# broadinstitute/gatk-bwamem-jni

Measured on AMD Instinct MI355X. Metric: 150bp reads aligned/sec vs GRCh38-scale reference (1/2/4/8 MI355X), higher is better.
Workload: dtype u8/int32/int64; 1 GPU; 10000000 x 150bp single-end synthetic reads per GPU vs synthetic GRCh38-scale genome (3100000000 bp, 24 contigs, 5% diverged repeats), full index in HBM; reads_per_gpu=10000000, read_len=150, genome_bp=3100000000, genome=iid, response_bytes=542940344, parallelism=read-sharded x1, no collectives, hip_hw_queues=4, paired_end=False

## Files before the change

### gatk-bwamem-jni_amd/csrc/bwamem_types.h

```cpp
#pragma once
#include <stdint.h>
#include <stddef.h>
#include <hip/hip_runtime.h>

struct MemOpt {
    int a, b;
    int o_del, e_del;
    int o_ins, e_ins;
    int pen_unpaired;
    int pen_clip5, pen_clip3;
    int w;
    int zdrop;
    uint64_t max_mem_intv;
    int T;
    int flag;
    int min_seed_len;
    int min_chain_weight;
    int max_chain_extend;
    float split_factor;
    int split_width;
    int max_occ;
    int max_chain_gap;
    int n_threads;
    int chunk_size;
    float mask_level;
    float drop_ratio;
    float XA_drop_ratio;
    float mask_level_redun;
    float mapQ_coef_len;
    int mapQ_coef_fac;
    int max_ins;
    int max_matesw;
    int max_XA_hits, max_XA_hits_alt;
    int8_t mat[25];
};
static_assert(sizeof(MemOpt) == 168, "mem_opt_t ABI (BwaMemAligner.java:137)");

struct MemPestat { int low, high; int failed; double avg, std; };
static_assert(sizeof(MemPestat) == 32, "mem_pestat_t ABI");

struct PairTab { const double* t; int64_t lo[4]; int32_t n[4], off[4]; };

enum {
    MEM_F_PE = 0x2, MEM_F_NOPAIRING = 0x4, MEM_F_ALL = 0x8, MEM_F_NO_MULTI = 0x10,
    MEM_F_NO_RESCUE = 0x20, MEM_F_PRIMARY5 = 0x800
};

struct DevIndex {
    const uint4* occ;
    const uint32_t* sa_lo;
    const uint8_t*  sa_hi;
    const uint8_t*  pac;
    const int64_t*  ann_offset;
    const int32_t*  ann_len;
    const int32_t*  ann_is_alt;
    const int32_t*  ann_name_off;
    const char*     names;
    const double*   log_tab;
    uint64_t primary, L2[5], seq_len;
    int64_t  l_pac;
    int32_t  n_seqs, sa_intv, log_tab_n, sa_shift;
    int32_t  n_cu, lds_bytes;
};

struct Intv { uint64_t x0, x1, size, info; };

struct Seed { int64_t rbeg; int32_t qbeg, len, score, next; };

struct Chain {
    int64_t pos;
    int32_t n, first, rid;
    uint32_t w;
    int32_t kept, is_alt;
    int32_t seed0;
    int32_t last;
    float frac_rep;
    int32_t pad_;
};

struct AlnReg {
    int64_t rb, re;
    int32_t qb, qe;
    int32_t rid;
    int32_t score, truesc, sub, alt_sc, csub, sub_n, w, seedcov, secondary, secondary_all, seedlen0;
    int32_t n_comp, is_alt;
    float frac_rep;
    int32_t pad_;
    uint64_t hash;
};

struct SwJob { int64_t rb; int32_t read, tag, l_ms, is_rev, tlen, xtra, q_off, pad_; };
struct KswR { int score, te, qe, score2, te2, tb, qb; };

struct DevCounters {
    unsigned long long n_ext, n_lf, n_sa, n_dp_cells, n_ref_bases, n_reads;
    unsigned long long dbg[10];
};

enum { ERR_INTV_CAP = 1, ERR_OUT_CAP = 2, ERR_CIGAR_CAP = 4, ERR_LONG_READ = 8, ERR_SCRATCH = 16, ERR_BTREE = 32, ERR_BAD_REG = 64, ERR_JOB_CAP = 128, ERR_ZPOOL = 256, ERR_RESCUE_CAP = 512 };

#define BT_NODE_INTS 40

struct TileView {
    int32_t n_reads;
    int32_t max_len;
    int64_t read_id0;
    const int64_t* seq_off;
    uint8_t* seq;
    int32_t intv_cap;
    Intv* intv;
    int32_t* n_intv;
    Intv* smem_scratch;
    int32_t smem_cap;
    int32_t* l_rep;
    int32_t* n_seeds;
    int64_t* seed_off;
// ... 31 lines not shown
```

### gatk-bwamem-jni_amd/csrc/k_seed.hip

```cpp
#include "dev_common.h"
#include "wave_ops.h"
#include "kernels.h"

DEV uint32_t mask16(int n)
{
    n = n < 0 ? 0 : n > 16 ? 16 : n;
    return (uint32_t)(0x5555555500000000ull >> (n << 1));
}
DEV void cnt_word_m(uint32_t x, uint32_t m, uint32_t& c1, uint32_t& c2, uint32_t& c3)
{
    const uint32_t lo = x & m, hi = (x >> 1) & m;
    c3 += __popc(hi & lo);
    c2 += __popc(hi & ~lo);
    c1 += __popc(~hi & lo);
}
DEV void extend_sm(const DevIndex& ix, uint64_t x0, uint64_t x1, uint64_t size, int c, bool is_back, uint64_t& o0, uint64_t& o1, uint64_t& osz)
{
    const uint64_t xa = is_back ? x0 : x1, xb = is_back ? x1 : x0;
    const uint64_t k = xa - 1, l = xa - 1 + size;
    const uint64_t kk = k - (k >= ix.primary), ll = l - (l >= ix.primary);
    const uint64_t bk = kk >> 6, bl = ll >> 6;
    const uint4* pk = ix.occ + 2 * bk;
    const uint4* pl = ix.occ + 2 * bl;
    const uint4 ck = pk[0], sk = pk[1], cl = pl[0], sl = pl[1];
// ... 23 lines not shown
    uint32_t *v0, *v1, *v2;
    uint16_t* v2n;
    uint4* spill;
    int K, spill_cap;
    bool narrow;
    static __device__ uint32_t pack2(uint64_t x0, uint64_t size, int end) { return (uint32_t)(x0 >> 32) | (uint32_t)(size >> 32) << 5 | (uint32_t)end << 10; }
    __device__ uint32_t hi_get(int e) const {
        const int s = (e & (K - 1)) * 64;
        if (!narrow) return v2[s];
        const uint32_t h = v2n[s];
        return (h & 7u) | (h >> 3 & 7u) << 5 | (h >> 6) << 10;
    }
    __device__ void hi_put(int e, uint32_t w2) {
        const int s = (e & (K - 1)) * 64;
        if (!narrow) v2[s] = w2;
        else v2n[s] = (uint16_t)((w2 & 7u) | (w2 >> 5 & 7u) << 3 | (w2 >> 10) << 6);
    }
    __device__ bool push(int e, uint64_t x0, uint64_t size, int end) {
        const int s = (e & (K - 1)) * 64;
        if (e >= K) {
            if (e - K >= spill_cap) return false;
            uint4 t; t.x = v0[s]; t.y = v1[s]; t.z = hi_get(e); t.w = 0;
            spill[(size_t)(e - K) * 64] = t;
        }
        v0[s] = (uint32_t)x0; v1[s] = (uint32_t)size; hi_put(e, pack2(x0, size, end));
        return true;
    }
    __device__ void put(int e, int n, uint64_t x0, uint64_t size, int end) {
        if (e >= n - K) { const int s = (e & (K - 1)) * 64; v0[s] = (uint32_t)x0; v1[s] = (uint32_t)size; hi_put(e, pack2(x0, size, end)); }
        else { uint4 t; t.x = (uint32_t)x0; t.y = (uint32_t)size; t.z = pack2(x0, size, end); t.w = 0; spill[(size_t)e * 64] = t; }
    }
    __device__ void get(int e, int n, uint64_t& x0, uint64_t& size, int& end) const {
        uint32_t a, b, w2;
        if (e >= n - K) { const int s = (e & (K - 1)) * 64; a = v0[s]; b = v1[s]; w2 = hi_get(e); }
        else { const uint4 t = spill[(size_t)e * 64]; a = t.x; b = t.y; w2 = t.z; }
        x0 = (uint64_t)(w2 & 31) << 32 | a; size = (uint64_t)(w2 >> 5 & 31) << 32 | b; end = (int)(w2 >> 10);
    }
};

__global__ void k_encode(uint8_t* seq, int64_t n_bytes)
{
    int64_t i = (int64_t)blockIdx.x * blockDim.x + threadIdx.x;
    int64_t stride = (int64_t)gridDim.x * blockDim.x;
    for (; i < n_bytes; i += stride) {
        uint8_t c = seq[i];
        if (c >= 4) {
            uint8_t u = c & 0xdf;
            c = u == 'A' ? 0 : u == 'C' ? 1 : u == 'G' ? 2 : u == 'T' ? 3 : 4;
            seq[i] = c;
        }
    }
}

enum { S_IDLE = 0, S_NEXT = 1, S_FWD = 2, S_BWD = 3, S_P3 = 4 };
#define SEED_EL_CAP 4

template <bool LDSQ>
__global__ void __launch_bounds__(64) k_seed(DevIndex ix, MemOpt opt, TileView tv, int K, int refill_min, int narrow)
{
    HIP_DYNAMIC_SHARED(uint32_t, lds)
    const int lane = threadIdx.x;
    CandStack V;
    V.narrow = narrow != 0;
    V.v0 = lds + lane; V.v1 = V.v0 + K * 64; V.v2 = V.v1 + K * 64; V.K = K;
    V.v2n = (uint16_t*)(lds + 2 * K * 64) + lane;
    V.spill = (uint4*)tv.smem_scratch + (size_t)blockIdx.x * tv.smem_cap * 64 + lane; V.spill_cap = tv.smem_cap;
    uint32_t* el = lds + (narrow ? 5 * K * 32 : 3 * K * 64) + lane;
    uint32_t* sq = el + SEED_EL_CAP * 64;
    unsigned int* work = (unsigned int*)(tv.err + 8);
    const int min_seed_len = opt.min_seed_len;
    const int split_len = (int)(opt.min_seed_len * opt.split_factor + .499);
    const uint64_t max_intv3 = (uint64_t)(int64_t)(int)opt.max_mem_intv;

    int st = S_IDLE, r = 0, len = 0, pass = 1, x = 0, sx = 0, i = 0, k2 = 0, old_n = 0, mem_n = 0;
    int nf = 0, lo = 0, rd = 0, wr = 0, c = -1, ret = 0, end = 0, n_el = 0;
    uint64_t min_intv = 1, last_start = 0, last_sz = 0, ik0 = 0, ik1 = 0, iks = 0;
    bool any = false, ovf = false, exhausted = false, el_ok = true;
    const uint8_t* qg = tv.seq;
    Intv* mem = tv.intv;
    uint32_t n_ext = 0;

    uint64_t qwin = 0;
    const uint8_t* qwin_at = nullptr;
    auto qat_g = [&](int p) -> int {
        const uint8_t* a = qg + p;
        const uint8_t* al = a - ((uintptr_t)a & 7);
        if (al != qwin_at) { qwin_at = al; qwin = *(const uint64_t*)al; }
        return (int)(qwin >> (((uintptr_t)a & 7) << 3) & 0xffu);
    };
#define QAT(p) (LDSQ ? (int)(sq[((p) >> 3) * 64] >> (((p) & 7) << 2) & 15u) : qat_g(p))
#define FINISH() do { fin = true; st = S_IDLE; } while (0)
#define MEM_PUSH(X0, SZ, INFO) do { if (mem_n >= tv.intv_cap) ovf = true; else { Intv v_; v_.x0 = (X0); v_.x1 = 0; v_.size = (SZ); v_.info = (INFO); mem[mem_n++] = v_; } } while (0)
#define PUSH_IK() do { if (V.push(nf, ik0, iks, end)) ++nf; else ovf = true; } while (0)
#define BEGIN_BWD() do { ret = end; lo = 0; rd = wr = nf - 1; i = sx - 1; c = i >= 0 ? QAT(i) : 4; c = c < 4 ? c : -1; st = S_BWD; } while (0)

    for (;;) {
        bool fin = false;
        const unsigned long long idle = __ballot(st == S_IDLE);
        if (idle != 0ull && !exhausted && (__popcll(idle) >= refill_min || idle == ~0ull)) {
            const int n_need = __popcll(idle);
            unsigned int base = 0;
            if (lane == 0) base = atomicAdd(work, (unsigned int)n_need);
            base = (unsigned int)__shfl((int)base, 0);
            if (base + (unsigned int)n_need >= (unsigned int)tv.n_reads) exhausted = true;
            bool fresh = false;
            if (st == S_IDLE) {
                const unsigned int cand = base + (unsigned int)__popcll(idle & ((1ull << lane) - 1ull));
                if (cand < (unsigned int)tv.n_reads) {
                    r = (int)cand; fresh = true;
                    const int64_t off = tv.seq_off[r];
                    len = (int)(tv.seq_off[r + 1] - off - 1);
                    qg = tv.seq + off;
                    mem = tv.intv + (size_t)r * tv.intv_cap;
                    mem_n = 0; ovf = false; pass = 1; x = 0; st = S_NEXT; n_el = 0; el_ok = true;
                }
            }
            if (LDSQ) {
                unsigned long long got = __ballot(fresh);
                while (got) {
                    const int l = __ffsll((long long)got) - 1;
                    got &= got - 1ull;
                    const int rr = __shfl(r, l);
                    const int64_t off = tv.seq_off[rr];
                    const int nb = (int)(tv.seq_off[rr + 1] - off) - 1;
                    for (int k = lane; k * 8 < nb; k += 64) {
                        uint32_t wd = 0;
                        uint32_t by[8];
#pragma unroll
                        for (int b = 0; b < 8; ++b) { const int pos = k * 8 + b; by[b] = tv.seq[off + (pos < nb ? pos : nb)]; }
#pragma unroll
                        for (int b = 0; b < 8; ++b) wd |= (k * 8 + b < nb ? by[b] & 15u : 4u) << (b << 2);
                        sq[k * 64 + (l - lane)] = wd;
                    }
                }
                __syncthreads();
            }
            if (fresh && len < min_seed_len) { tv.n_intv[r] = 0; st = S_IDLE; }
        }
        if (__ballot(st != S_IDLE) == 0ull) break;

        if (st == S_NEXT) {
            int nx = -1;
            bool p3 = false;
            uint64_t nmin = 1;
            if (pass == 1) {
                if (x >= len) { pass = 2; old_n = mem_n; k2 = 0; }
                else if (QAT(x) > 3) ++x;
                else nx = x;
            } else if (pass == 2 && el_ok) {
                if (k2 >= n_el) { pass = 3; x = 0; if (!(opt.max_mem_intv > 0)) FINISH(); }
                else {
                    const uint32_t wd = el[k2 * 64];
                    const int m = (int)(wd & 0x1ffffu);
                    if (QAT(m) > 3) ++k2;
                    else { nx = m; nmin = (uint64_t)(wd >> 17) + 1; }
                }
            } else if (pass == 2) {
                if (k2 >= old_n) { pass = 3; x = 0; if (!(opt.max_mem_intv > 0)) FINISH(); }
                else {
                    const uint64_t psz = mem[k2].size, pinfo = mem[k2].info;
                    const int s0 = (int)(pinfo >> 32), e0 = (int)(int32_t)pinfo;
                    if (e0 - s0 < split_len || psz > (uint64_t)(int64_t)opt.split_width) ++k2;
                    else {
                        const int m = (s0 + e0) >> 1;
                        if (QAT(m) > 3) ++k2;
                        else { nx = m; nmin = psz + 1; }
                    }
                }
            } else {
                if (x >= len) FINISH();
                else if (QAT(x) > 3) ++x;
                else { nx = x; p3 = true; }
            }
            if (nx >= 0) {
                const int b = QAT(nx);
                const uint64_t lb = b == 0 ? ix.L2[0] : b == 1 ? ix.L2[1] : b == 2 ? ix.L2[2] : ix.L2[3];
                const uint64_t lb1 = b == 0 ? ix.L2[1] : b == 1 ? ix.L2[2] : b == 2 ? ix.L2[3] : ix.L2[4];
                const uint64_t lc = b == 0 ? ix.L2[3] : b == 1 ? ix.L2[2] : b == 2 ? ix.L2[1] : ix.L2[0];
                ik0 = lb + 1; iks = lb1 - lb; ik1 = lc + 1;
                sx = nx; i = sx + 1;
                if (p3) st = S_P3;
                else { min_intv = nmin; end = sx + 1; nf = 0; any = false; st = S_FWD; }
            }
        }

        bool need = false, bw = false, back = false;
        int rc = 0, pend = 0;
        uint64_t r0 = 0, r1 = 0, rs = 0;
        bool fwd_end = false;
        if (st == S_FWD || st == S_P3) {
            const int cq = i < len ? QAT(i) : 4;
            if (cq < 4) { need = true; rc = 3 - cq; r0 = ik0; r1 = ik1; rs = iks; }
            else if (st == S_FWD) fwd_end = true;
            else { x = i < len ? i + 1 : len; st = S_NEXT; }
        }
        if (st == S_BWD) {
            V.get(rd, nf, r0, rs, pend);
            bw = true;
            if (c >= 0) { need = true; back = true; rc = c; }
        }

        uint64_t o0 = 0, o1 = 0, os = 0, em0 = 0, ems = 0, emi = 0;
        bool emit = false;
        if (need) { extend_sm(ix, r0, r1, rs, rc, back, o0, o1, os); ++n_ext; }

        if (bw) {
            if (!need || os < min_intv) {
                if (wr == nf - 1 && (!any || (uint64_t)(i + 1) < last_start)) {
                    any = true; last_start = (uint64_t)(i + 1);
                    if (pend - (i + 1) >= min_seed_len) {
                        emit = true; em0 = r0; ems = rs; emi = (uint64_t)(i + 1) << 32 | (uint32_t)pend;
                        if (pass == 1 && pend - (i + 1) >= split_len && rs <= (uint64_t)(int64_t)opt.split_width) {
                            if (n_el < SEED_EL_CAP && rs < 32768u) el[n_el * 64] = (uint32_t)((i + 1 + pend) >> 1) | (uint32_t)rs << 17;
                            else el_ok = false;
                            ++n_el;
                        }
                    }
                }
            } else if (wr == nf - 1 || os != last_sz) {
                V.put(wr, nf, o0, os, pend); --wr; last_sz = os;
            }
            --rd;
            if (rd < lo) {
                if (wr == nf - 1) { if (pass == 1) x = ret; else ++k2; st = S_NEXT; }
                else { lo = wr + 1; rd = wr = nf - 1; --i; c = i >= 0 ? QAT(i) : 4; c = c < 4 ? c : -1; }
            }
        } else if (st == S_FWD && (need || fwd_end)) {
            const bool push = fwd_end || os != iks;
            const bool stop = fwd_end || (push && os < min_intv);
            if (push) PUSH_IK();
            if (stop) BEGIN_BWD();
            else { ik0 = o0; ik1 = o1; iks = os; end = i + 1; ++i; }
        } else if (need) {
            if (os < max_intv3 && i - sx >= min_seed_len) {
                if (os > 0) { emit = true; em0 = o0; ems = os; emi = (uint64_t)sx << 32 | (uint32_t)(i + 1); }
                x = i + 1; st = S_NEXT;
            } else { ik0 = o0; ik1 = o1; iks = os; ++i; }
        }
        if (emit) MEM_PUSH(em0, ems, emi);
        if (ovf) FINISH();
        if (fin) {
            tv.n_intv[r] = ovf ? 0 : mem_n;
            if (ovf) atomicOr(tv.err, ERR_INTV_CAP);
        }
    }
#undef QAT
#undef FINISH
#undef MEM_PUSH
#undef PUSH_IK
#undef BEGIN_BWD
    unsigned long long tot = n_ext;
    for (int o = 32; o > 0; o >>= 1) tot += __shfl_down(tot, o);
    if (lane == 0) { count_add(&tv.cnt->n_ext, tot); }
}

__global__ void k_seed_fin(MemOpt opt, TileView tv)
{
    const int r = blockIdx.x * blockDim.x + threadIdx.x;
    if (r >= tv.n_reads) return;
    Intv* a = tv.intv + (size_t)r * tv.intv_cap;
    const int n = tv.n_intv[r];
    for (int i = 1; i < n; ++i) {
        Intv t = a[i];
        int j = i;
        while (j > 0 && a[j - 1].info > t.info) { a[j] = a[j - 1]; --j; }
        a[j] = t;
    }
    int n_seeds = 0, l_rep = 0, b = 0, e = 0;
    int32_t* iso = tv.intv_seed_off + (size_t)r * tv.intv_cap;
    for (int i = 0; i < n; ++i) {
        const Intv p = a[i];
        const int sb = (int)(p.info >> 32), se = (int)(uint32_t)p.info;
        iso[i] = n_seeds;
        {
            int64_t step = p.size > (uint64_t)(int64_t)opt.max_occ ? (int64_t)(p.size / (uint64_t)opt.max_occ) : 1;
            int64_t c = ((int64_t)p.size + step - 1) / step;
            n_seeds += (int)(c < opt.max_occ ? c : opt.max_occ);
        }
        if (p.size <= (uint64_t)(int64_t)opt.max_occ) continue;
        if (sb > e) { l_rep += e - b; b = sb; e = se; }
        else e = e > se ? e : se;
    }
    l_rep += e - b;
    tv.n_seeds[r] = n_seeds;
    tv.l_rep[r] = l_rep;
}

__global__ void __launch_bounds__(1024) k_scan(const int32_t* in, int64_t* out, int n)
{
    __shared__ int64_t wtot[2][16];
    const int t = threadIdx.x, lane = t & 63, wv = t >> 6;
    int64_t carry = 0;
    int ph = 0;
    for (int base = 0; base < n; base += 4096, ph ^= 1) {
        const int i0 = base + t * 4;
        int v0 = 0, v1 = 0, v2 = 0, v3 = 0;
        if (i0 + 3 < n) { const int4 q = *(const int4*)(in + i0); v0 = q.x; v1 = q.y; v2 = q.z; v3 = q.w; }
        else { if (i0 < n) v0 = in[i0]; if (i0 + 1 < n) v1 = in[i0 + 1]; if (i0 + 2 < n) v2 = in[i0 + 2]; }
        const int64_t sum = (int64_t)v0 + v1 + v2 + v3;
        int64_t incl = sum;
        for (int o = 1; o < 64; o <<= 1) { int64_t u = __shfl_up(incl, o); if (lane >= o) incl += u; }
        if (lane == 63) wtot[ph][wv] = incl;
        __syncthreads();
        int64_t pre = carry, tot = 0;
        for (int w = 0; w < 16; ++w) { const int64_t x = wtot[ph][w]; if (w < wv) pre += x; tot += x; }
        int64_t run = pre + incl - sum;
        if (i0 < n) out[i0] = run;
        run += v0; if (i0 + 1 < n) out[i0 + 1] = run;
        run += v1; if (i0 + 2 < n) out[i0 + 2] = run;
        run += v2; if (i0 + 3 < n) out[i0 + 3] = run;
        carry += tot;
    }
    if (t == 0) out[n] = carry;
}

DEV int64_t block_excl_scan_256(int64_t v, int64_t* lds4, int64_t& total)
{
    const int lane = threadIdx.x & 63, wv = threadIdx.x >> 6;
    int64_t incl = v;
    for (int o = 1; o < 64; o <<= 1) { int64_t u = __shfl_up(incl, o); if (lane >= o) incl += u; }
    if (lane == 63) lds4[wv] = incl;
    __syncthreads();
// ... 274 lines not shown
```

### gatk-bwamem-jni_amd/csrc/kernels.h

```cpp
#pragma once
#include <hip/hip_runtime.h>
#include "bwamem_types.h"
#include "bam_encode.h"
#include "bam_sort.h"
#include "bam_dup.h"
#include "fastq_parse.h"

void launch_build_occ64(hipStream_t st, const uint32_t* bwt, uint64_t n_blocks, uint4* occ);
void launch_sa_densify(hipStream_t st, const DevIndex& ix, const uint64_t* sa_src, uint64_t n_src, int src_intv, uint32_t* lo, uint8_t* hi, int32_t* err);
void launch_encode(hipStream_t st, uint8_t* seq, int64_t n_bytes);
void launch_unpack_pac(hipStream_t st, const DevIndex& ix, int64_t start, int64_t n, uint8_t* dst);
void launch_seed(hipStream_t st, const DevIndex& ix, const MemOpt& opt, const TileView& tv);
size_t scan_tmp_bytes(int64_t n);
void launch_scan(hipStream_t st, const int32_t* in, int64_t* out, int n, int64_t* tmp);
void launch_order(hipStream_t st, const int32_t* n_seeds, int n, int32_t* bins64, int32_t* order);
size_t nul_tmp_bytes(int64_t n_bytes);
void launch_nul_offsets(hipStream_t st, const uint8_t* seq, int64_t n_bytes, int64_t* off, int64_t n_reads_max, int64_t* n_found, void* tmp);
void launch_sa(hipStream_t st, const DevIndex& ix, const MemOpt& opt, const TileView& tv, int64_t n_occ);
void launch_chain(hipStream_t st, const DevIndex& ix, const MemOpt& opt, const TileView& tv, Chain* chain_store);
bool rescore_needed(const MemOpt& opt, const TileView& tv);
void launch_rescore(hipStream_t st, const DevIndex& ix, const MemOpt& opt, const TileView& tv, void* jobs, void* results, int32_t* first_num, int32_t* cnt, int cap);
size_t extend_lds_bytes(const MemOpt& opt, int max_len);
void launch_extend(hipStream_t st, const DevIndex& ix, const MemOpt& opt, const TileView& tv);
void launch_post1(hipStream_t st, const DevIndex& ix, const MemOpt& opt, const TileView& tv);
void launch_final_prep(hipStream_t st, const DevIndex& ix, const MemOpt& opt, const TileView& tv);
size_t gcigar_slab_bytes(const MemOpt& opt, int max_len);
int gcigar_slab_grid(const DevIndex& ix, int n_jobs);
void launch_gcigar(hipStream_t st, const DevIndex& ix, const MemOpt& opt, const TileView& tv, int n_jobs, const void* jobs, void* outs, uint32_t* cig_pool, int cig_cap,
                   uint8_t* zpool, unsigned long long zpool_cap, unsigned long long* zpool_cur, uint8_t* slabs, size_t slab_bytes, int* queue);
void launch_final_se(hipStream_t st, const DevIndex& ix, const MemOpt& opt, const TileView& tv, const void* job_out, const uint32_t* job_cig, int cig_cap);
void launch_pack(hipStream_t st, const TileView& tv, uint8_t* dst);
void launch_bam_size(hipStream_t st, const BamTile& t);
void launch_bam_emit(hipStream_t st, const BamTile& t);
void launch_qual_check(hipStream_t st, const uint8_t* raw, const uint8_t* qual, const int64_t* raw_off, int n_reads, int32_t* err);
void launch_mate_names(hipStream_t st, const uint8_t* names, const int64_t* name_off, int n_pairs, int32_t* err);
void launch_fastq_count(hipStream_t st, const uint8_t* text, int64_t n, int32_t* counts);
void launch_fastq_starts(hipStream_t st, const FastqText& t);
void launch_fastq_records(hipStream_t st, const FastqText& t, const FastqOut& o);
void launch_fastq_copy(hipStream_t st, const FastqText& t, const FastqOut& o, int max_len);
int bgzf_grid(int n_cu, int64_t n_blocks);
size_t bgzf_token_bytes(int grid);
void launch_bgzf_deflate(hipStream_t st, const uint8_t* src, int64_t n, int n_blocks, int grid, uint8_t* slots, int32_t* sizes, uint32_t* tokens);
void launch_bgzf_gather(hipStream_t st, const uint8_t* slots, const int32_t* sizes, const int64_t* off, int n_blocks, bool with_eof, uint8_t* out);
void launch_sort_bits(hipStream_t st, const uint64_t* keys, int64_t n, int32_t* bits);
void launch_sort_hist(hipStream_t st, const uint64_t* keys, int64_t n, int byte, int32_t* hist);
void launch_sort_scatter(hipStream_t st, const uint64_t* keys, const uint32_t* idx, int64_t n, int byte, const int64_t* off, uint64_t* keys_out, uint32_t* idx_out);
void launch_bamrec_count(hipStream_t st, const uint8_t* bam, const int64_t* bam_off, int n_reads, int32_t* counts, int32_t* bits, int32_t* err);
void launch_bamrec_keys(hipStream_t st, const uint8_t* bam, const int64_t* bam_off, int n_reads, const int64_t* first, uint64_t* keys, int64_t* src_off, int32_t* sizes);
void launch_bamrec_sizes(hipStream_t st, const uint32_t* idx, const int32_t* sizes, int n, int32_t* out);
void launch_bamrec_gather(hipStream_t st, const uint8_t* src, const int64_t* src_off, const uint32_t* idx, const int64_t* dst_off, int n_rec, int64_t total, uint8_t* dst);
void launch_bai_records(hipStream_t st, const BaiView& v);
void launch_bai_mark(hipStream_t st, const uint64_t* keys, const uint32_t* idx, int n, int32_t* start);
void launch_bai_chunks(hipStream_t st, const uint64_t* keys, const uint32_t* idx, int n, const int32_t* start, const int64_t* cid, const int64_t* rec_off,
                       const int64_t* member_off, int64_t coffset0, BaiChunk* out);
void launch_bai_windows(hipStream_t st, const int32_t* win, int n_win, int n_rec, const int64_t* rec_off, const int64_t* member_off, int64_t coffset0, uint64_t* out);
void launch_dup_entries(hipStream_t st, const DupView& v);
void launch_dup_scores(hipStream_t st, const DupView& v, int max_len);
void launch_dup_score_keys(hipStream_t st, const DupView& v, uint64_t* frag_key, uint64_t* pair_key);
void launch_dup_gather(hipStream_t st, const uint64_t* src, const uint32_t* idx, int n, uint64_t* out);
void launch_dup_decide(hipStream_t st, const uint64_t* keys, const uint32_t* idx, const uint64_t* second, int n, const uint8_t* is_paired, uint8_t* dup);
void launch_dup_flags(hipStream_t st, const DupView& v);

void launch_pestat_cand(hipStream_t st, const DevIndex& ix, const MemOpt& opt, const TileView& tv, int8_t* cand_dir, int64_t* cand_is);
void launch_pe_caps(hipStream_t st, const MemOpt& opt, const TileView& tv, int32_t* caps);
// ... 10 lines not shown
```

### gatk-bwamem-jni_amd/csrc/pipeline.cpp

```cpp
#include <hip/hip_runtime.h>
#include <stdio.h>
#include <stdlib.h>
#include <string.h>
#include <math.h>
#include <unistd.h>
#include <fcntl.h>
#include <errno.h>
#include <time.h>
#include <sys/stat.h>
#include <sys/mman.h>
#include <dlfcn.h>
#include <mutex>
#include <condition_variable>
#include <thread>
#include <atomic>
#include <functional>
#include <memory>
#include <string>
#include <vector>
#include <deque>
#include <stdexcept>
#include <algorithm>
#include <cmath>
#include "bwamem_types.h"
// ... 139 lines not shown
    }
};

struct ReqBuf {
    DevBuf seq, off, tmp;
    int64_t* h_off = nullptr; size_t h_cap = 0;
    ~ReqBuf() { if (h_off) (void)hipHostFree(h_off); }
    bool ensure_host(size_t n) {
        if (n <= h_cap) return true;
        if (h_off) (void)hipHostFree(h_off);
        h_off = nullptr; h_cap = 0;
        n += n / 8 + 64;
        if (hipHostMalloc((void**)&h_off, n * 8, hipHostMallocDefault) != hipSuccess) { h_off = nullptr; return false; }
        h_cap = n;
        return true;
    }
};

struct CapHints {
    std::mutex mu;
    double jobs_per_read = 0, zpool_mult = 1;
    double seeds_per_read = 0;
    int out_cap = 512;
    void saw_seeds(int T, int64_t n_occ) { std::lock_guard<std::mutex> lk(mu); if (T >= 1024) seeds_per_read = seeds_per_read == 0 ? (double)n_occ / T : 0.75 * seeds_per_read + 0.25 * (double)n_occ / T; }
    int tile_scale() { std::lock_guard<std::mutex> lk(mu); return seeds_per_read > 32 ? 2 : 1; }
    void learn(int T, int n_jobs, double zpool_mult_, int out_cap_) {
        std::lock_guard<std::mutex> lk(mu);
        if (T >= 64) jobs_per_read = std::max(jobs_per_read, 1.25 * n_jobs / T);
        zpool_mult = std::min(64.0, std::max(zpool_mult, zpool_mult_));
        out_cap = std::max(out_cap, out_cap_);
    }
    void get(int T, int& jobs, double& zpool_mult_, int& out_cap_) {
        std::lock_guard<std::mutex> lk(mu);
        jobs = (int)std::min(1.0e9, jobs_per_read * T) + 1; zpool_mult_ = zpool_mult; out_cap_ = out_cap;
    }
    double pe_rescue_per_read = 0, pe_jobs_per_read = 0;
    int pe_cap_u = 256;
    void learn_pe(int T, int n_rescue, int n_jobs, int cap_u) {
        std::lock_guard<std::mutex> lk(mu);
        if (T >= 64) { pe_rescue_per_read = std::max(pe_rescue_per_read, 1.25 * n_rescue / T); pe_jobs_per_read = std::max(pe_jobs_per_read, 1.25 * n_jobs / T); }
        pe_cap_u = std::min(2048, std::max(pe_cap_u, cap_u));
    }
    void get_pe(int T, int& rescue, int& jobs, int& cap_u) {
        std::lock_guard<std::mutex> lk(mu);
        rescue = (int)std::min(1.0e9, pe_rescue_per_read * T) + 1; jobs = (int)std::min(1.0e9, pe_jobs_per_read * T) + 1; cap_u = pe_cap_u;
    }
};

struct bwaidx_s {
    uint8_t* mem = nullptr; size_t l_mem = 0; bool mmapped = false;
    HostIndex h;
    int device = 0;
    DevIndex d;
    DevBuf d_occ, d_sa_lo, d_sa_hi, d_pac, d_ann_off, d_ann_len, d_ann_alt, d_name_off, d_names, d_log, d_ptab;
    PairTab pair_tab;
    std::mutex mu;
    Workspace ws;
    std::vector<std::unique_ptr<Workspace>> extra_ws;
    Workspace seed_ws;
    SeedStore seed_store[SEED_STORES_MAX];
    CapHints hints;
    std::vector<std::unique_ptr<ReqBuf>> req_bufs;
    hipStream_t up_stream = nullptr;
    std::vector<bwaidx_s*> peers;
    std::atomic<uint32_t> next_replica{0};
    std::mutex split_mu;
    ~bwaidx_s() { if (up_stream) (void)hipStreamDestroy(up_stream); }
};

struct TileOut {
    uint8_t* d = nullptr; size_t bytes = 0; bool owned = false;
    int64_t* d_off = nullptr; int64_t read_id = 0; int n_reads = 0, max_len = 0;
};

struct PeTile { uint32_t r0 = 0; int T = 0, L = 0; uint8_t* seq = nullptr; const int64_t* seq_off = nullptr; DevBuf n_regs, regs, reg_off; int64_t n_regs_total = 0; std::vector<int8_t> cand_dir; std::vector<int64_t> cand_is; };
struct PeCall { std::deque<PeTile> tiles; int64_t read_id0 = 0; };

struct OutSink {
    bool to_host = false;
    std::mutex mu; std::condition_variable cv;
    std::deque<int64_t> bytes, start;
    size_t n_placed = 0; int64_t placed_end = 0;
    uint64_t reads_total = 0, reads_known = 0;
    uint8_t* h_buf = nullptr; size_t h_cap = 0; int inflight = 0;
    DevBuf pool; size_t last_total = 0;
    bool aborted = false;
    void begin_call(uint64_t n_reads) {
        std::lock_guard<std::mutex> lk(mu);
        bytes.clear(); start.clear(); n_placed = 0; placed_end = 0; reads_total = n_reads; reads_known = 0; inflight = 0; aborted = false;
        if (h_buf) { free(h_buf); h_buf = nullptr; } h_cap = 0;
    }
    void add_tiles(size_t n) { std::lock_guard<std::mutex> lk(mu); bytes.resize(bytes.size() + n, -1); start.resize(start.size() + n, 0); }
    void abort() { { std::lock_guard<std::mutex> lk(mu); aborted = true; } cv.notify_all(); }
    bool place(size_t i, int64_t nbytes, int n_reads, uint8_t** dst) {
        std::unique_lock<std::mutex> lk(mu);
        bytes[i] = nbytes; reads_known += (uint64_t)n_reads;
        cv.notify_all();
        cv.wait(lk, [&] {
            while (n_placed < bytes.size() && bytes[n_placed] >= 0) { start[n_placed] = placed_end; placed_end += bytes[n_placed]; ++n_placed; }
            return aborted || n_placed > i;
        });
        if (aborted) return false;
        const size_t need = (size_t)(start[i] + nbytes);
        if (!to_host) { *dst = pool.p && need <= pool.bytes ? pool.as<uint8_t>() + start[i] : nullptr; return true; }
        if (need > h_cap) {
            cv.wait(lk, [&] { return aborted || inflight == 0; });
            if (aborted) return false;
// ... 78 lines not shown
    if (!ix->d_pac.ensure((size_t)(h.l_pac / 4 + 1) + 16)) return false;
    HIP_OK(hipMemcpy(ix->d_pac.p, h.pac, (size_t)(h.l_pac / 4 + 1), hipMemcpyHostToDevice));
    std::vector<int64_t> off(n); std::vector<int32_t> len(n), alt(n), noff(n + 1);
    std::string names;
    for (int i = 0; i < n; ++i) {
        off[i] = h.contigs[i].offset; len[i] = h.contigs[i].len; alt[i] = h.contigs[i].is_alt;
        noff[i] = (int32_t)names.size();
        names += h.contigs[i].name; names.push_back('\0');
    }
    noff[n] = (int32_t)names.size();
    if (!ix->d_ann_off.ensure((size_t)n * 8 + 8) || !ix->d_ann_len.ensure((size_t)n * 4 + 4) || !ix->d_ann_alt.ensure((size_t)n * 4 + 4)
        || !ix->d_name_off.ensure((size_t)(n + 1) * 4) || !ix->d_names.ensure(names.size() + 1) || !ix->d_log.ensure((size_t)LOG_TAB_N * 8)) return false;
    HIP_OK(hipMemcpy(ix->d_ann_off.p, off.data(), (size_t)n * 8, hipMemcpyHostToDevice));
    HIP_OK(hipMemcpy(ix->d_ann_len.p, len.data(), (size_t)n * 4, hipMemcpyHostToDevice));
    HIP_OK(hipMemcpy(ix->d_ann_alt.p, alt.data(), (size_t)n * 4, hipMemcpyHostToDevice));
    HIP_OK(hipMemcpy(ix->d_name_off.p, noff.data(), (size_t)(n + 1) * 4, hipMemcpyHostToDevice));
    HIP_OK(hipMemcpy(ix->d_names.p, names.data(), names.size(), hipMemcpyHostToDevice));
    {
        std::vector<double> lt(LOG_TAB_N);
        for (int i = 0; i < LOG_TAB_N; ++i) lt[i] = log((double)i);
        HIP_OK(hipMemcpy(ix->d_log.p, lt.data(), (size_t)LOG_TAB_N * 8, hipMemcpyHostToDevice));
    }
    DevIndex& d = ix->d;
    memset(&d, 0, sizeof d);
    d.occ = ix->d_occ.as<uint4>(); d.pac = ix->d_pac.as<uint8_t>();
    d.ann_offset = ix->d_ann_off.as<int64_t>(); d.ann_len = ix->d_ann_len.as<int32_t>(); d.ann_is_alt = ix->d_ann_alt.as<int32_t>();
    d.ann_name_off = ix->d_name_off.as<int32_t>(); d.names = ix->d_names.as<char>(); d.log_tab = ix->d_log.as<double>();
    d.primary = h.primary; for (int i = 0; i < 5; ++i) d.L2[i] = h.L2[i];
    d.seq_len = h.seq_len; d.l_pac = h.l_pac; d.n_seqs = n; d.log_tab_n = LOG_TAB_N;
    {
        int v = 0;
        d.n_cu = hipDeviceGetAttribute(&v, hipDeviceAttributeMultiprocessorCount, ix->device) == hipSuccess && v > 0 ? v : 256;
        d.lds_bytes = hipDeviceGetAttribute(&v, hipDeviceAttributeMaxSharedMemoryPerBlock, ix->device) == hipSuccess && v > 0 ? v : 64 << 10;
    }
    {
        int dense = 1;
        if (const char* e = getenv("BWAMEM_HIP_SA_INTV")) { dense = atoi(e); if (dense < 1 || (dense & (dense - 1))) dense = 1; }
        size_t free_b = 0, total_b = 0;
        HIP_OK(hipMemGetInfo(&free_b, &total_b));
        if (dense > h.sa_intv) dense = h.sa_intv;
        while (dense < h.sa_intv && ((size_t)(h.seq_len / dense) + 1) * 5 + (size_t)h.n_sa * 8 > free_b / 4) dense <<= 1;
        d.sa_intv = dense; d.sa_shift = 0;
        while ((1 << d.sa_shift) < dense) ++d.sa_shift;
        const size_t n_kept = (size_t)(h.seq_len >> d.sa_shift) + 1;
        DevBuf src, flag;
        if (!ix->d_sa_lo.ensure(n_kept * 4 + 64) || !ix->d_sa_hi.ensure(n_kept + 64) || !src.ensure((size_t)h.n_sa * 8) || !flag.ensure(64)) return false;
        d.sa_lo = ix->d_sa_lo.as<uint32_t>(); d.sa_hi = ix->d_sa_hi.as<uint8_t>();
        int32_t bad = 1;
        if (hipMemcpy(src.p, h.sa, (size_t)h.n_sa * 8, hipMemcpyHostToDevice) == hipSuccess && hipMemset(flag.p, 0, 64) == hipSuccess) {
            launch_sa_densify(0, d, src.as<uint64_t>(), h.n_sa, h.sa_intv, ix->d_sa_lo.as<uint32_t>(), ix->d_sa_hi.as<uint8_t>(), flag.as<int32_t>());
            if (hipDeviceSynchronize() != hipSuccess || hipMemcpy(&bad, flag.p, 4, hipMemcpyDeviceToHost) != hipSuccess) bad = 1;
        }
        if (bad) { fprintf(stderr, "[bwamem_hip] suffix array densification failed\n"); return false; }
    }
    return true;
}

struct Roctx {
    int (*push)(const char*) = nullptr; int (*pop)() = nullptr;
    Roctx() {
        if (const char* e = getenv("BWAMEM_HIP_ROCTX")) if (atoi(e) == 0) return;
        for (const char* lib : { "librocprofiler-sdk-roctx.so", "librocprofiler-sdk-roctx.so.1", "libroctx64.so", "libroctx64.so.4" }) {
            void* h = dlopen(lib, RTLD_LAZY | RTLD_LOCAL);
            if (!h) continue;
            push = (int (*)(const char*))dlsym(h, "roctxRangePushA"); pop = (int (*)())dlsym(h, "roctxRangePop");
            if (push && pop) return;
            push = nullptr; pop = nullptr;
        }
    }
};
static Roctx& roctx() { static Roctx r; return r; }
struct RoctxRange { bool on; RoctxRange(const char* name) : on(roctx().push != nullptr) { if (on) roctx().push(name); } ~RoctxRange() { if (on) roctx().pop(); } };

static void timed_begin(Workspace& ws, KernelId id)
{
    if (!g_stats.enabled) return;
    Timed t; t.id = id;
    if (hipEventCreate(&t.a) != hipSuccess || hipEventCreate(&t.b) != hipSuccess) return;
    (void)hipEventRecord(t.a, ws.stream);
    ws.timed.push_back(t);
}
static void timed_end(Workspace& ws)
{
    if (!g_stats.enabled || ws.timed.empty()) return;
    (void)hipEventRecord(ws.timed.back().b, ws.stream);
}
static void timed_collect(Workspace& ws)
{
    if (ws.timed.empty()) return;
    std::lock_guard<std::mutex> lk(g_stats.mu);
    for (Timed& t : ws.timed) {
        float ms = 0;
        if (hipEventElapsedTime(&ms, t.a, t.b) == hipSuccess) {
            double* slot[K_N] = { &g_stats.s.ms_encode, &g_stats.s.ms_seed, &g_stats.s.ms_sa, &g_stats.s.ms_chain, &g_stats.s.ms_extend,
                                  &g_stats.s.ms_post, &g_stats.s.ms_final, &g_stats.s.ms_pack, &g_stats.s.ms_other };
            *slot[t.id] += ms;
            if (t.id == K_SEED) ++g_stats.s.n_launch_seed;
            if (t.id == K_SA) ++g_stats.s.n_launch_sa;
            if (t.id == K_EXTEND) ++g_stats.s.n_launch_extend;
        }
        (void)hipEventDestroy(t.a); (void)hipEventDestroy(t.b);
    }
    ws.timed.clear();
}
static int g_verbose = -1;
static bool verbose() { if (g_verbose < 0) { const char* e = getenv("BWAMEM_HIP_VERBOSE"); g_verbose = e && atoi(e) > 0; } return g_verbose > 0; }
// ... 1928 lines not shown
```

Baseline: 23.19 million reads/s.

## Split third seeding pass into separate sweep with k-mer interval lookup table

Builds a table of precomputed SA intervals for all 12-mers at index load time. The third (reseeding) pass of SMEM finding now runs as its own work-claiming sweep after passes 1 and 2, and starts each forward extension from a table lookup instead of k single-base FM-index extensions. Pass-3 results are written to the tail of the per-read interval buffer and merged in the post-processing kernel. This cuts occurrence-table lookups and divergence from mixing pass-3 lanes with pass-1/2 lanes, at the cost of a 256 MiB table, a second read claim and a merge step.

Result: slower. 21.70 million reads/s (-6.4%).

```diff
diff --git a/gatk-bwamem-jni_amd/csrc/bwamem_types.h b/gatk-bwamem-jni_amd/csrc/bwamem_types.h
--- a/gatk-bwamem-jni_amd/csrc/bwamem_types.h
+++ b/gatk-bwamem-jni_amd/csrc/bwamem_types.h
@@ -61,7 +61,11 @@
     int64_t  l_pac;
     int32_t  n_seqs, sa_intv, log_tab_n, sa_shift;
     int32_t  n_cu, lds_bytes;
+    const uint4* kmer_tab;
+    int32_t  kmer_k;
 };
+
+#define SEED_KMER_MAX 13
 
 struct Intv { uint64_t x0, x1, size, info; };
 
diff --git a/gatk-bwamem-jni_amd/csrc/k_seed.hip b/gatk-bwamem-jni_amd/csrc/k_seed.hip
--- a/gatk-bwamem-jni_amd/csrc/k_seed.hip
+++ b/gatk-bwamem-jni_amd/csrc/k_seed.hip
@@ -99,6 +99,44 @@
     }
 }
 
+DEV uint4 kmer_pack(uint64_t x0, uint64_t x1, uint64_t size)
+{
+    uint4 e;
+    e.x = (uint32_t)x0; e.y = (uint32_t)x1; e.z = (uint32_t)size;
+    e.w = (uint32_t)(x0 >> 32 & 31) | (uint32_t)(x1 >> 32 & 31) << 5 | (uint32_t)(size >> 32 & 31) << 10;
+    return e;
+}
+DEV void kmer_unpack(const uint4 e, uint64_t& x0, uint64_t& x1, uint64_t& size)
+{
+    x0 = (uint64_t)(e.w & 31) << 32 | e.x; x1 = (uint64_t)(e.w >> 5 & 31) << 32 | e.y; size = (uint64_t)(e.w >> 10 & 31) << 32 | e.z;
+}
+DEV void base_intv(const DevIndex& ix, int b, uint64_t& x0, uint64_t& x1, uint64_t& size)
+{
+    const uint64_t lb = b == 0 ? ix.L2[0] : b == 1 ? ix.L2[1] : b == 2 ? ix.L2[2] : ix.L2[3];
+    const uint64_t lb1 = b == 0 ? ix.L2[1] : b == 1 ? ix.L2[2] : b == 2 ? ix.L2[3] : ix.L2[4];
+    const uint64_t lc = b == 0 ? ix.L2[3] : b == 1 ? ix.L2[2] : b == 2 ? ix.L2[1] : ix.L2[0];
+    x0 = lb + 1; size = lb1 - lb; x1 = lc + 1;
+}
+__global__ void __launch_bounds__(256) k_build_kmer(DevIndex ix, int k, uint4* tab)
+{
+    const uint64_t t = (uint64_t)blockIdx.x * blockDim.x + threadIdx.x;
+    if (t >> (2 * k)) return;
+    uint64_t x0, x1, sz;
+    base_intv(ix, (int)(t & 3), x0, x1, sz);
+    for (int j = 1; j < k; ++j) {
+        uint64_t o0, o1, os;
+        extend_sm(ix, x0, x1, sz, 3 - (int)(t >> (2 * j) & 3), false, o0, o1, os);
+        x0 = o0; x1 = o1; sz = os;
+    }
+    tab[t] = kmer_pack(x0, x1, sz);
+}
+void launch_build_kmer(hipStream_t st, const DevIndex& ix, int k, uint4* tab)
+{
+    if (k < 1 || k > SEED_KMER_MAX) return;
+    const uint64_t n = 1ull << (2 * k);
+    hipLaunchKernelGGL(k_build_kmer, dim3((unsigned)((n + 255) / 256)), dim3(256), 0, st, ix, k, tab);
+}
+
 enum { S_IDLE = 0, S_NEXT = 1, S_FWD = 2, S_BWD = 3, S_P3 = 4 };
 #define SEED_EL_CAP 4
 
@@ -114,7 +152,6 @@
     V.spill = (uint4*)tv.smem_scratch + (size_t)blockIdx.x * tv.smem_cap * 64 + lane; V.spill_cap = tv.smem_cap;
     uint32_t* el = lds + (narrow ? 5 * K * 32 : 3 * K * 64) + lane;
     uint32_t* sq = el + SEED_EL_CAP * 64;
-    unsigned int* work = (unsigned int*)(tv.err + 8);
     const int min_seed_len = opt.min_seed_len;
     const int split_len = (int)(opt.min_seed_len * opt.split_factor + .499);
     const uint64_t max_intv3 = (uint64_t)(int64_t)(int)opt.max_mem_intv;
@@ -135,6 +172,47 @@
         if (al != qwin_at) { qwin_at = al; qwin = *(const uint64_t*)al; }
         return (int)(qwin >> (((uintptr_t)a & 7) << 3) & 0xffu);
     };
+    auto claim = [&](unsigned int* work) -> bool {
+        const unsigned long long idle = __ballot(st == S_IDLE);
+        if (!(idle != 0ull && !exhausted && (__popcll(idle) >= refill_min || idle == ~0ull))) return false;
+        const int n_need = __popcll(idle);
+        unsigned int base = 0;
+        if (lane == 0) base = atomicAdd(work, (unsigned int)n_need);
+        base = (unsigned int)__shfl((int)base, 0);
+        if (base + (unsigned int)n_need >= (unsigned int)tv.n_reads) exhausted = true;
+        bool fresh = false;
+        if (st == S_IDLE) {
+            const unsigned int cand = base + (unsigned int)__popcll(idle & ((1ull << lane) - 1ull));
+            if (cand < (unsigned int)tv.n_reads) {
+                r = (int)cand; fresh = true;
+                const int64_t off = tv.seq_off[r];
+                len = (int)(tv.seq_off[r + 1] - off - 1);
+                qg = tv.seq + off;
+                mem = tv.intv + (size_t)r * tv.intv_cap;
+            }
+        }
+        if (LDSQ) {
+            unsigned long long got = __ballot(fresh);
+            while (got) {
+                const int l = __ffsll((long long)got) - 1;
+                got &= got - 1ull;
+                const int rr = __shfl(r, l);
+                const int64_t off = tv.seq_off[rr];
+                const int nb = (int)(tv.seq_off[rr + 1] - off) - 1;
+                for (int k = lane; k * 8 < nb; k += 64) {
+                    uint32_t wd = 0;
+                    uint32_t by[8];
+#pragma unroll
+                    for (int b = 0; b < 8; ++b) { const int pos = k * 8 + b; by[b] = tv.seq[off + (pos < nb ? pos : nb)]; }
+#pragma unroll
+                    for (int b = 0; b < 8; ++b) wd |= (k * 8 + b < nb ? by[b] & 15u : 4u) << (b << 2);
+                    sq[k * 64 + (l - lane)] = wd;
+                }
+            }
+            __syncthreads();
+        }
+        return fresh;
+    };
 #define QAT(p) (LDSQ ? (int)(sq[((p) >> 3) * 64] >> (((p) & 7) << 2) & 15u) : qat_g(p))
 #define FINISH() do { fin = true; st = S_IDLE; } while (0)
 #define MEM_PUSH(X0, SZ, INFO) do { if (mem_n >= tv.intv_cap) ovf = true; else { Intv v_; v_.x0 = (X0); v_.x1 = 0; v_.size = (SZ); v_.info = (INFO); mem[mem_n++] = v_; } } while (0)
@@ -143,91 +221,42 @@
 
     for (;;) {
         bool fin = false;
-        const unsigned long long idle = __ballot(st == S_IDLE);
-        if (idle != 0ull && !exhausted && (__popcll(idle) >= refill_min || idle == ~0ull)) {
-            const int n_need = __popcll(idle);
-            unsigned int base = 0;
-            if (lane == 0) base = atomicAdd(work, (unsigned int)n_need);
-            base = (unsigned int)__shfl((int)base, 0);
-            if (base + (unsigned int)n_need >= (unsigned int)tv.n_reads) exhausted = true;
-            bool fresh = false;
-            if (st == S_IDLE) {
-                const unsigned int cand = base + (unsigned int)__popcll(idle & ((1ull << lane) - 1ull));
-                if (cand < (unsigned int)tv.n_reads) {
-                    r = (int)cand; fresh = true;
-                    const int64_t off = tv.seq_off[r];
-                    len = (int)(tv.seq_off[r + 1] - off - 1);
-                    qg = tv.seq + off;
-                    mem = tv.intv + (size_t)r * tv.intv_cap;
-                    mem_n = 0; ovf = false; pass = 1; x = 0; st = S_NEXT; n_el = 0; el_ok = true;
-                }
-            }
-            if (LDSQ) {
-                unsigned long long got = __ballot(fresh);
-                while (got) {
-                    const int l = __ffsll((long long)got) - 1;
-                    got &= got - 1ull;
-                    const int rr = __shfl(r, l);
-                    const int64_t off = tv.seq_off[rr];
-                    const int nb = (int)(tv.seq_off[rr + 1] - off) - 1;
-                    for (int k = lane; k * 8 < nb; k += 64) {
-                        uint32_t wd = 0;
-                        uint32_t by[8];
-#pragma unroll
-                        for (int b = 0; b < 8; ++b) { const int pos = k * 8 + b; by[b] = tv.seq[off + (pos < nb ? pos : nb)]; }
-#pragma unroll
-                        for (int b = 0; b < 8; ++b) wd |= (k * 8 + b < nb ? by[b] & 15u : 4u) << (b << 2);
-                        sq[k * 64 + (l - lane)] = wd;
-                    }
-                }
-                __syncthreads();
-            }
-            if (fresh && len < min_seed_len) { tv.n_intv[r] = 0; st = S_IDLE; }
-        }
-        if (__ballot(st != S_IDLE) == 0ull) break;
+        if (claim((unsigned int*)(tv.err + 8))) {
+            mem_n = 0; ovf = false; pass = 1; x = 0; st = S_NEXT; n_el = 0; el_ok = true;
+            if (len < min_seed_len) { tv.n_intv[r] = 0; st = S_IDLE; }
+        }
+        if (__ballot(st != S_IDLE) == 0ull) { if (exhausted) break; continue; }
 
         if (st == S_NEXT) {
             int nx = -1;
-            bool p3 = false;
             uint64_t nmin = 1;
             if (pass == 1) {
                 if (x >= len) { pass = 2; old_n = mem_n; k2 = 0; }
                 else if (QAT(x) > 3) ++x;
                 else nx = x;
-            } else if (pass == 2 && el_ok) {
-                if (k2 >= n_el) { pass = 3; x = 0; if (!(opt.max_mem_intv > 0)) FINISH(); }
+            } else if (el_ok) {
+                if (k2 >= n_el) FINISH();
                 else {
                     const uint32_t wd = el[k2 * 64];
                     const int m = (int)(wd & 0x1ffffu);
                     if (QAT(m) > 3) ++k2;
                     else { nx = m; nmin = (uint64_t)(wd >> 17) + 1; }
                 }
-            } else if (pass == 2) {
-                if (k2 >= old_n) { pass = 3; x = 0; if (!(opt.max_mem_intv > 0)) FINISH(); }
+            } else {
+                if (k2 >= old_n) FINISH();
                 else {
                     const uint64_t psz = mem[k2].size, pinfo = mem[k2].info;
                     const int s0 = (int)(pinfo >> 32), e0 = (int)(int32_t)pinfo;
-                    if (e0 - s0 < split_len || psz > (uint64_t)(int64_t)opt.split_width) ++k2;
-                    else {
-                        const int m = (s0 + e0) >> 1;
-                        if (QAT(m) > 3) ++k2;
-                        else { nx = m; nmin = psz + 1; }
-                    }
+                    const int m = (int)(((uint32_t)s0 + (uint32_t)e0) >> 1);
+                    if ((int64_t)e0 - s0 < split_len || psz > (uint64_t)(int64_t)opt.split_width || m >= len) ++k2;
+                    else if (QAT(m) > 3) ++k2;
+                    else { nx = m; nmin = psz + 1; }
                 }
-            } else {
-                if (x >= len) FINISH();
-                else if (QAT(x) > 3) ++x;
-                else { nx = x; p3 = true; }
             }
             if (nx >= 0) {
-                const int b = QAT(nx);
-                const uint64_t lb = b == 0 ? ix.L2[0] : b == 1 ? ix.L2[1] : b == 2 ? ix.L2[2] : ix.L2[3];
-                const uint64_t lb1 = b == 0 ? ix.L2[1] : b == 1 ? ix.L2[2] : b == 2 ? ix.L2[3] : ix.L2[4];
-                const uint64_t lc = b == 0 ? ix.L2[3] : b == 1 ? ix.L2[2] : b == 2 ? ix.L2[1] : ix.L2[0];
-                ik0 = lb + 1; iks = lb1 - lb; ik1 = lc + 1;
+                base_intv(ix, QAT(nx), ik0, ik1, iks);
                 sx = nx; i = sx + 1;
-                if (p3) st = S_P3;
-                else { min_intv = nmin; end = sx + 1; nf = 0; any = false; st = S_FWD; }
+                min_intv = nmin; end = sx + 1; nf = 0; any = false; st = S_FWD;
             }
         }
 
@@ -235,11 +264,10 @@
         int rc = 0, pend = 0;
         uint64_t r0 = 0, r1 = 0, rs = 0;
         bool fwd_end = false;
-        if (st == S_FWD || st == S_P3) {
+        if (st == S_FWD) {
             const int cq = i < len ? QAT(i) : 4;
             if (cq < 4) { need = true; rc = 3 - cq; r0 = ik0; r1 = ik1; rs = iks; }
-            else if (st == S_FWD) fwd_end = true;
-            else { x = i < len ? i + 1 : len; st = S_NEXT; }
+            else fwd_end = true;
         }
         if (st == S_BWD) {
             V.get(rd, nf, r0, rs, pend);
@@ -247,7 +275,7 @@
             if (c >= 0) { need = true; back = true; rc = c; }
         }
 
-        uint64_t o0 = 0, o1 = 0, os = 0, em0 = 0, ems = 0, emi = 0;
+        uint64_t o0 = 0, o1 = 0, os = 0;
         bool emit = false;
         if (need) { extend_sm(ix, r0, r1, rs, rc, back, o0, o1, os); ++n_ext; }
 
@@ -256,7 +284,7 @@
                 if (wr == nf - 1 && (!any || (uint64_t)(i + 1) < last_start)) {
                     any = true; last_start = (uint64_t)(i + 1);
                     if (pend - (i + 1) >= min_seed_len) {
-                        emit = true; em0 = r0; ems = rs; emi = (uint64_t)(i + 1) << 32 | (uint32_t)pend;
+                        emit = true;
                         if (pass == 1 && pend - (i + 1) >= split_len && rs <= (uint64_t)(int64_t)opt.split_width) {
                             if (n_el < SEED_EL_CAP && rs < 32768u) el[n_el * 64] = (uint32_t)((i + 1 + pend) >> 1) | (uint32_t)rs << 17;
                             else el_ok = false;
@@ -268,27 +296,83 @@
                 V.put(wr, nf, o0, os, pend); --wr; last_sz = os;
             }
             --rd;
-            if (rd < lo) {
+            if (rd < lo || c < 0) {
                 if (wr == nf - 1) { if (pass == 1) x = ret; else ++k2; st = S_NEXT; }
                 else { lo = wr + 1; rd = wr = nf - 1; --i; c = i >= 0 ? QAT(i) : 4; c = c < 4 ? c : -1; }
             }
-        } else if (st == S_FWD && (need || fwd_end)) {
+        } else if (st == S_FWD) {
             const bool push = fwd_end || os != iks;
             const bool stop = fwd_end || (push && os < min_intv);
             if (push) PUSH_IK();
             if (stop) BEGIN_BWD();
             else { ik0 = o0; ik1 = o1; iks = os; end = i + 1; ++i; }
-        } else if (need) {
-            if (os < max_intv3 && i - sx >= min_seed_len) {
-                if (os > 0) { emit = true; em0 = o0; ems = os; emi = (uint64_t)sx << 32 | (uint32_t)(i + 1); }
-                x = i + 1; st = S_NEXT;
-            } else { ik0 = o0; ik1 = o1; iks = os; ++i; }
-        }
-        if (emit) MEM_PUSH(em0, ems, emi);
+        }
+        if (emit) MEM_PUSH(r0, rs, (uint64_t)(i + 1) << 32 | (uint32_t)pend);
         if (ovf) FINISH();
         if (fin) {
-            tv.n_intv[r] = ovf ? 0 : mem_n;
+            tv.n_intv[r] = ovf ? -1 : mem_n;
             if (ovf) atomicOr(tv.err, ERR_INTV_CAP);
+        }
+    }
+
+    {
+        st = S_IDLE; exhausted = false;
+        const bool p3_on = opt.max_mem_intv > 0;
+        const int kmer_k = ix.kmer_tab && ix.kmer_k >= 1 && ix.kmer_k <= SEED_KMER_MAX && ix.kmer_k <= min_seed_len ? ix.kmer_k : 0;
+        int n3 = 0;
+        for (;;) {
+            if (claim((unsigned int*)(tv.err + 9))) {
+                n3 = 0; x = 0; st = S_NEXT;
+                if (len < min_seed_len || !p3_on) { tv.intv_seed_off[(size_t)r * tv.intv_cap] = 0; st = S_IDLE; }
+            }
+            if (__ballot(st != S_IDLE) == 0ull) { if (exhausted) break; continue; }
+            bool fin = false;
+            if (st == S_NEXT) {
+                if (x + min_seed_len >= len) fin = true;
+                else {
+                    bool jump = false;
+                    uint32_t km = 0;
+                    if (kmer_k > 0 && x + kmer_k <= len) {
+                        if (LDSQ) {
+                            const int wi = x >> 3, wl = (len - 1) >> 3, sh = (x & 7) << 2;
+                            const uint32_t w0 = sq[wi * 64], w1 = sq[(wi + 1 < wl ? wi + 1 : wl) * 64], w2 = sq[(wi + 2 < wl ? wi + 2 : wl) * 64];
+                            uint64_t v = (uint64_t)w1 << 32 | w0;
+                            if (sh) v = v >> sh | (uint64_t)w2 << (64 - sh);
+                            v &= ~0ull >> (64 - 4 * kmer_k);
+                            jump = !(v & 0x4444444444444444ull);
+                            v = (v | v >> 2) & 0x0f0f0f0f0f0f0f0full;
+                            v = (v | v >> 4) & 0x00ff00ff00ff00ffull;
+                            v = (v | v >> 8) & 0x0000ffff0000ffffull;
+                            km = (uint32_t)(v | v >> 16);
+                        } else {
+                            uint32_t bad = 0;
+                            for (int j = 0; j < kmer_k; ++j) { const uint32_t b = (uint32_t)QAT(x + j); bad |= b; km |= (b & 3u) << (2 * j); }
+                            jump = bad < 4u;
+                        }
+                    }
+                    if (jump) { kmer_unpack(ix.kmer_tab[km], ik0, ik1, iks); sx = x; i = x + kmer_k; st = S_P3; }
+                    else {
+                        const int b = QAT(x);
+                        if (b > 3) ++x;
+                        else { base_intv(ix, b, ik0, ik1, iks); sx = x; i = x + 1; st = S_P3; }
+                    }
+                }
+            }
+            if (st == S_P3) {
+                const int cq = i < len ? QAT(i) : 4;
+                if (cq < 4) {
+                    uint64_t o0, o1, os;
+                    extend_sm(ix, ik0, ik1, iks, 3 - cq, false, o0, o1, os); ++n_ext;
+                    if (os < max_intv3 && i - sx >= min_seed_len) {
+                        if (os > 0) {
+                            if (n3 >= tv.intv_cap) { n3 = tv.intv_cap + 1; fin = true; }
+                            else { Intv v_; v_.x0 = o0; v_.x1 = 0; v_.size = os; v_.info = (uint64_t)sx << 32 | (uint32_t)(i + 1); mem[tv.intv_cap - 1 - n3] = v_; ++n3; }
+                        }
+                        x = i + 1; st = S_NEXT;
+                    } else { ik0 = o0; ik1 = o1; iks = os; ++i; }
+                } else { x = i < len ? i + 1 : len; st = S_NEXT; }
+            }
+            if (fin) { tv.intv_seed_off[(size_t)r * tv.intv_cap] = n3; st = S_IDLE; }
         }
     }
 #undef QAT
@@ -305,8 +389,20 @@
 {
     const int r = blockIdx.x * blockDim.x + threadIdx.x;
     if (r >= tv.n_reads) return;
-    Intv* a = tv.intv + (size_t)r * tv.intv_cap;
-    const int n = tv.n_intv[r];
+    const int cap = tv.intv_cap;
+    Intv* a = tv.intv + (size_t)r * cap;
+    int32_t* iso = tv.intv_seed_off + (size_t)r * cap;
+    const int n12 = tv.n_intv[r], n3 = iso[0];
+    int n = 0;
+    if (n12 < 0 || n3 < 0 || n3 > cap || n12 + n3 > cap) atomicOr(tv.err, ERR_INTV_CAP);
+    else {
+        if (n12 + n3 > cap - n3) {
+            for (int j = 0; 2 * j + 1 < n3; ++j) { const Intv t = a[cap - 1 - j]; a[cap - 1 - j] = a[cap - n3 + j]; a[cap - n3 + j] = t; }
+            if (n12 < cap - n3) for (int j = 0; j < n3; ++j) a[n12 + j] = a[cap - n3 + j];
+        } else for (int j = 0; j < n3; ++j) a[n12 + j] = a[cap - 1 - j];
+        n = n12 + n3;
+    }
+    tv.n_intv[r] = n;
     for (int i = 1; i < n; ++i) {
         Intv t = a[i];
         int j = i;
@@ -314,7 +410,6 @@
         a[j] = t;
     }
     int n_seeds = 0, l_rep = 0, b = 0, e = 0;
-    int32_t* iso = tv.intv_seed_off + (size_t)r * tv.intv_cap;
     for (int i = 0; i < n; ++i) {
         const Intv p = a[i];
         const int sb = (int)(p.info >> 32), se = (int)(uint32_t)p.info;
diff --git a/gatk-bwamem-jni_amd/csrc/kernels.h b/gatk-bwamem-jni_amd/csrc/kernels.h
--- a/gatk-bwamem-jni_amd/csrc/kernels.h
+++ b/gatk-bwamem-jni_amd/csrc/kernels.h
@@ -10,6 +10,7 @@
 void launch_sa_densify(hipStream_t st, const DevIndex& ix, const uint64_t* sa_src, uint64_t n_src, int src_intv, uint32_t* lo, uint8_t* hi, int32_t* err);
 void launch_encode(hipStream_t st, uint8_t* seq, int64_t n_bytes);
 void launch_unpack_pac(hipStream_t st, const DevIndex& ix, int64_t start, int64_t n, uint8_t* dst);
+void launch_build_kmer(hipStream_t st, const DevIndex& ix, int k, uint4* tab);
 void launch_seed(hipStream_t st, const DevIndex& ix, const MemOpt& opt, const TileView& tv);
 size_t scan_tmp_bytes(int64_t n);
 void launch_scan(hipStream_t st, const int32_t* in, int64_t* out, int n, int64_t* tmp);
diff --git a/gatk-bwamem-jni_amd/csrc/pipeline.cpp b/gatk-bwamem-jni_amd/csrc/pipeline.cpp
--- a/gatk-bwamem-jni_amd/csrc/pipeline.cpp
+++ b/gatk-bwamem-jni_amd/csrc/pipeline.cpp
@@ -215,7 +215,7 @@
     HostIndex h;
     int device = 0;
     DevIndex d;
-    DevBuf d_occ, d_sa_lo, d_sa_hi, d_pac, d_ann_off, d_ann_len, d_ann_alt, d_name_off, d_names, d_log, d_ptab;
+    DevBuf d_occ, d_sa_lo, d_sa_hi, d_pac, d_ann_off, d_ann_len, d_ann_alt, d_name_off, d_names, d_log, d_ptab, d_kmer;
     PairTab pair_tab;
     std::mutex mu;
     Workspace ws;
@@ -400,6 +400,20 @@
             if (hipDeviceSynchronize() != hipSuccess || hipMemcpy(&bad, flag.p, 4, hipMemcpyDeviceToHost) != hipSuccess) bad = 1;
         }
         if (bad) { fprintf(stderr, "[bwamem_hip] suffix array densification failed\n"); return false; }
+    }
+    {
+        int k = 12;
+        const char* e = getenv("BWAMEM_HIP_SEED_KMER");
+        if (e && atoi(e) >= 0 && atoi(e) <= SEED_KMER_MAX) k = atoi(e);
+        else while (k > 1 && (1ull << (2 * k)) > h.seq_len) --k;
+        size_t free_b = 0, total_b = 0;
+        HIP_OK(hipMemGetInfo(&free_b, &total_b));
+        const size_t bytes = k > 0 ? (size_t)16 << (2 * k) : 0;
+        if (k > 0 && bytes <= free_b / 8 && ix->d_kmer.ensure(bytes)) {
+            launch_build_kmer(0, d, k, ix->d_kmer.as<uint4>());
+            HIP_OK(hipDeviceSynchronize());
+            d.kmer_tab = ix->d_kmer.as<uint4>(); d.kmer_k = k;
+        }
     }
     return true;
 }
```
